# Takatsuka-Mark/Photogrammetry

Hardware: AMD Instinct MI355X
Metric: descriptor pairs matched/sec (higher is better)
Workload: dtype u8 / bits (descriptor bits expanded to fp4 +-1 for the MFMA distance: exact integers in f32 accumulators; integer keys); f32 grey; 1 GPU; BASELINE configs[2] (SURVEY 8d config 3) x 1: 64-frame 1920x1080 RGBA64 sequence(s), dewarp(shipped coeffs)+gray+FAST(T=0.1)+NMS(r=16; SURVEY 8d writes r = 20 for this config: both leave more than 4096 survivors per frame, the lists are cut to the same length either way)+BRIEF-256 per frame, all 2016 ordered image pairs per sequence through the greedy Hamming match, <=4096 keypoints per frame (fir; frames=64, image_pairs=2016, frames_per_gpu=64, image_pairs_per_gpu=2016, parallelism=frames f mod 1, image pairs p mod 1; 2 all-gathers per step (elided at N = 1), jobs_in_flight=2, rehearsal_on_one_gpu_with_gloo=False

## Files before the change

### photogrammetry_amd/csrc/k_brief.hip

```cpp
#include "pgx_internal.h"

namespace {

constexpr int MAX_WORDS = 128;

__device__ __forceinline__ void brief_256(const float *__restrict__ g, int W, int H, int x, int y,
                                          const int4 *__restrict__ pairs, uint32_t *__restrict__ out)
{
    const int lane = threadIdx.x & 63;
    int4 pr[4];
#pragma unroll
    for (int c = 0; c < 4; c++) pr[c] = pairs[c * 64 + lane];
    float v1[4], v2[4];
    bool ok[4];
#pragma unroll
    for (int c = 0; c < 4; c++) {
        const int x1 = x + pr[c].x, y1 = y + pr[c].y, x2 = x + pr[c].z, y2 = y + pr[c].w;
        ok[c] = x1 >= 0 && x1 < W && y1 >= 0 && y1 < H && x2 >= 0 && x2 < W && y2 >= 0 && y2 < H;
        v1[c] = ok[c] ? g[(size_t)y1 * W + x1] : 0.f;
        v2[c] = ok[c] ? g[(size_t)y2 * W + x2] : 0.f;
    }
    unsigned long long rev[4];
#pragma unroll
    for (int c = 0; c < 4; c++) rev[c] = __brevll(__ballot(ok[c] && v1[c] < v2[c]));
    if (lane < 8) {
        const int q = lane >> 1;
        const unsigned long long r = q == 0 ? rev[3] : (q == 1 ? rev[2] : (q == 2 ? rev[1] : rev[0]));
        out[lane] = (lane & 1) ? (uint32_t)(r >> 32) : (uint32_t)r;
    }
}

__device__ __forceinline__ void brief_one(const float *__restrict__ g, int W, int H, int x, int y,
                                          const int4 *__restrict__ pairs, int P, int words, uint32_t *wbuf ,
                                          uint32_t *__restrict__ out)
{
    const int lane = threadIdx.x & 63;
    for (int w = lane; w < words + 2; w += 64) wbuf[w] = 0;
    __builtin_amdgcn_wave_barrier();
    const int nchunk = (P + 63) / 64;
    for (int c = 0; c < nchunk; c++) {
        const int p = c * 64 + lane;
        bool bit = false;
        if (p < P) {
            const int4 pr = pairs[p];
            const int x1 = x + pr.x, y1 = y + pr.y;
            if (x1 >= 0 && x1 < W && y1 >= 0 && y1 < H) {
                const int x2 = x + pr.z, y2 = y + pr.w;
                if (x2 >= 0 && x2 < W && y2 >= 0 && y2 < H)
                    bit = g[(size_t)y1 * W + x1] < g[(size_t)y2 * W + x2];
            }
        }
        const unsigned long long rev = __brevll(__ballot(bit));
        if (lane == 0) {
            const int off = P - 64 * (c + 1);
            unsigned long long v = rev;
            int o = off;
            if (o < 0) { v >>= -o; o = 0; }
            const int wi = o >> 5, sh = o & 31;
            wbuf[wi] |= (uint32_t)(v << sh);
            wbuf[wi + 1] |= (uint32_t)(sh ? (v >> (32 - sh)) : (v >> 32));
            if (sh) wbuf[wi + 2] |= (uint32_t)(v >> (64 - sh));
        }
    }
    __builtin_amdgcn_wave_barrier();
    for (int w = lane; w < words; w += 64) out[w] = wbuf[w];
}

__global__ __launch_bounds__(256) void k_brief_kept(const float *__restrict__ gray, int W, int H,
                                                    const uint32_t *__restrict__ raw_xy,
                                                    const int32_t *__restrict__ raw_score, int raw_cap,
                                                    const uint32_t *__restrict__ order,
                                                    const int32_t *__restrict__ n_kept, int kp_cap,
                                                    const int4 *__restrict__ pairs, int P, int words,
                                                    pgx_keypoint *__restrict__ kp_out, uint32_t *__restrict__ desc_out,
                                                    int32_t *__restrict__ counts_out, int nframes, int out_stride)
{
    __shared__ uint32_t wbuf[4][MAX_WORDS + 2];
    const int nblk = (kp_cap + 3) / 4;
    const int F8 = (nframes / 8) * 8;
    int f, kb;
    {
        const int Lid = blockIdx.x;
        if (Lid < nblk * F8) {
            const int j = Lid >> 3;
            f = (j / nblk) * 8 + (Lid & 7);
            kb = j % nblk;
        } else {
            const int r = Lid - nblk * F8;
            f = F8 + r / nblk;
            kb = r % nblk;
        }
    }
    const int wv = threadIdx.x >> 6, lane = threadIdx.x & 63;
    const int k = kb * 4 + wv;
    const int nk = n_kept[f];
    if (kb == 0 && threadIdx.x == 0) counts_out[f] = nk;
    if (k >= nk) return;
    const uint32_t ri = order[(size_t)f * kp_cap + k];
    const uint32_t xy = raw_xy[(size_t)f * raw_cap + ri];
    const int x = (int)(xy & 0xFFFFu), y = (int)(xy >> 16);
    const float *g = gray + (size_t)f * W * H;
    if (lane == 0) {
        pgx_keypoint kp;
        kp.x = x; kp.y = y; kp.fast_score = raw_score[(size_t)f * raw_cap + ri];
        kp.value = g[(size_t)y * W + x];
        kp_out[(size_t)f * out_stride + k] = kp;
    }
    if (P == 256) brief_256(g, W, H, x, y, pairs, desc_out + ((size_t)f * out_stride + k) * 8);
    else brief_one(g, W, H, x, y, pairs, P, words, wbuf[wv], desc_out + ((size_t)f * out_stride + k) * words);
}

__global__ __launch_bounds__(256) void k_brief_list(const float *__restrict__ gray, int W, int H,
                                                    const pgx_keypoint *__restrict__ kps, int n,
                                                    const int4 *__restrict__ pairs, int P, int words,
                                                    uint32_t *__restrict__ desc_out)
{
    __shared__ uint32_t wbuf[4][MAX_WORDS + 2];
    const int wv = threadIdx.x >> 6;
    const int k = blockIdx.x * 4 + wv;
    if (k >= n) return;
    if (P == 256) brief_256(gray, W, H, kps[k].x, kps[k].y, pairs, desc_out + (size_t)k * 8);
    else brief_one(gray, W, H, kps[k].x, kps[k].y, pairs, P, words, wbuf[wv], desc_out + (size_t)k * words);
}

}

void pgx_launch_brief(hipStream_t s, const float *gray, int F, int W, int H, const uint32_t *raw_xy,
                      const int32_t *raw_score, int raw_cap, const uint32_t *order, const int32_t *n_kept,
                      int kp_cap, const int32_t *pairs, int P, pgx_keypoint *kp_out, uint32_t *desc_out,
                      int32_t *counts_out, int out_stride)
{
    if (F <= 0 || kp_cap <= 0) return;
    const int words = (P + 31) / 32;
    hipLaunchKernelGGL(k_brief_kept, dim3(((kp_cap + 3) / 4) * F), dim3(256), 0, s, gray, W, H, raw_xy, raw_score,
                       raw_cap, order, n_kept, kp_cap, reinterpret_cast<const int4 *>(pairs), P, words, kp_out,
                       desc_out, counts_out, F, out_stride);
}

void pgx_launch_brief_list(hipStream_t s, const float *gray, int W, int H, const pgx_keypoint *kps, int n,
                           const int32_t *pairs, int P, uint32_t *desc_out)
{
    if (n <= 0) return;
    const int words = (P + 31) / 32;
    hipLaunchKernelGGL(k_brief_list, dim3((n + 3) / 4), dim3(256), 0, s, gray, W, H, kps, n,
                       reinterpret_cast<const int4 *>(pairs), P, words, desc_out);
}
```

### photogrammetry_amd/csrc/pgx_api.hip

```cpp
#include "pgx_trackgraph.h"

#include <atomic>
#include <cmath>
#include <cstdarg>
#include <cstdio>
#include <new>
#include <cstring>
#include <cstdlib>

#define PGX_VERSION_STR "pgx 0.1 (gfx950)"

static thread_local std::string tl_err;
static thread_local const pgx_ctx *tl_err_ctx = nullptr;
static thread_local unsigned long long tl_err_id = 0;
static std::atomic<unsigned long long> g_ctx_ids{0};

void pgx_note_error(pgx_ctx *c, const std::string &msg)
{
    tl_err = msg;
    tl_err_ctx = c;
    tl_err_id = c ? c->id : 0;
    if (c) {
        std::lock_guard<std::mutex> g(c->err_mu);
        c->err = msg;
    }
}

namespace {

int fail(pgx_ctx *c, int code, const char *fmt, ...)
{
    char buf[512];
    va_list ap;
    va_start(ap, fmt);
    vsnprintf(buf, sizeof buf, fmt, ap);
    va_end(ap);
    pgx_note_error(c, buf);
    return code;
}

#define HIPCHK(c, expr)                                                                           \
    do {                                                                                          \
        hipError_t e_ = (expr);                                                                   \
        if (e_ != hipSuccess) return fail((c), PGX_E_HIP, "%s: %s", #expr, hipGetErrorString(e_)); \
    } while (0)

struct Lock {
    std::lock_guard<std::mutex> g;
    explicit Lock(pgx_ctx *c) : g(c->mu) { (void)hipSetDevice(c->device); }
};

int decode_status(pgx_ctx *c, int bits)
{
// ... 61 lines not shown
    if (dims_ok(c, W, H) != PGX_OK) return PGX_E_BADARG;
    if (c->map_set && (c->mapW != W || c->mapH != H))
        return fail(c, PGX_E_DIM_MISMATCH, "image %dx%d vs dewarp map %dx%d (ArgumentException)", W, H, c->mapW, c->mapH);
    if (F <= 0) return PGX_OK;
    const size_t npix = (size_t)W * H;
    const size_t nseg = pgx_fast_seg_count(W, H);
    const int raw_cap = c->raw_cap;
    HIPCHK(c, c->ws_gray.ensure((size_t)F * npix * 4));
    HIPCHK(c, c->ws_seg.ensure((size_t)F * nseg * 32));
    HIPCHK(c, c->ws_segoff.ensure((size_t)F * nseg * 4));
    HIPCHK(c, c->ws_rawxy.ensure((size_t)F * raw_cap * 4));
    HIPCHK(c, c->ws_rawscore.ensure((size_t)F * raw_cap * 4));
    const size_t nms_stride = pgx_nms_ws_bytes(W, H, c->radius, raw_cap, true);
    HIPCHK(c, c->ws_nms.ensure((size_t)F * nms_stride));
    const int kp_eff = c->kp_cap <= cap ? c->kp_cap : cap;
    HIPCHK(c, c->ws_order.ensure((size_t)F * kp_eff * 4));
    HIPCHK(c, c->ws_nkept.ensure((size_t)F * 4));
    return PGX_OK;
}

int pgx_enqueue_detect(pgx_ctx *c, const uint16_t *d_rgba, int F, int W, int H, pgx_keypoint *d_kp, uint32_t *d_desc,
                       int32_t *d_counts, int32_t *d_nraw, int cap)
{
    const int rcp = pgx_prepare_detect(c, F, W, H, cap);
    if (rcp != PGX_OK) return rcp;
    if (F <= 0) return PGX_OK;
    const int raw_cap = c->raw_cap;
    const size_t nms_stride = pgx_nms_ws_bytes(W, H, c->radius, raw_cap, true);
    const bool kp_soft = c->kp_cap <= cap;
    const int kp_eff = kp_soft ? c->kp_cap : cap;

    float *gray = c->ws_gray.as<float>();
    {
        ProfScope ps(c, "dewarp_gray");
        pgx_launch_dewarp_gray(c->stream, d_rgba, c->src8, c->map_set ? c->d_map.as<int32_t>() : nullptr, F, W, H, gray,
                               nullptr, c->d_status);
    }
    {
        ProfScope ps(c, "fast");
        pgx_launch_fast(c->stream, gray, F, W, H, c->threshold, c->ws_seg.as<unsigned long long>(),
                        c->ws_segoff.as<uint32_t>(), d_nraw, c->ws_rawxy.as<uint32_t>(),
                        c->ws_rawscore.as<int32_t>(), raw_cap, c->d_status,
                        !pgx_nms_fills_raw_lists(W, H, c->radius, raw_cap));
    }
    {
        ProfScope ps(c, "nms");
        pgx_launch_nms(c->stream, c->ws_rawxy.as<uint32_t>(), c->ws_rawscore.as<int32_t>(), d_nraw, F, raw_cap, W, H,
                       c->radius, c->ws_nms.p, nms_stride, c->ws_order.as<uint32_t>(), c->ws_nkept.as<int32_t>(),
                       kp_eff, c->d_status, c->ws_seg.as<unsigned long long>(), c->ws_segoff.as<uint32_t>(), kp_soft);
    }
    {
        ProfScope ps(c, "brief");
        pgx_launch_brief(c->stream, gray, F, W, H, c->ws_rawxy.as<uint32_t>(), c->ws_rawscore.as<int32_t>(), raw_cap,
                         c->ws_order.as<uint32_t>(), c->ws_nkept.as<int32_t>(), kp_eff, c->d_pairs.as<int32_t>(), c->P,
                         d_kp, d_desc, d_counts, cap);
    }
    HIPCHK(c, hipEventRecord(c->ev_stage[PGX_STAGE_DETECT], c->stream));
    HIPCHK(c, hipGetLastError());
    return PGX_OK;
}

int pgx_prepare_match(pgx_ctx *c, int stride, int words, int M)
{
    if (M <= 0) return PGX_OK;
    if (stride <= 0 || stride > (1 << PGX_IDX_BITS)) return fail(c, PGX_E_BADARG, "stride must be in [1, 2^20]");
    if (words <= 0 || words > 127) return fail(c, PGX_E_BADARG, "words must be in [1, 127] (P <= 4064)");
    const int CHUNK = c->match_chunk;
    const int mc = M < CHUNK ? M : CHUNK;
    const int nws = (M <= CHUNK || c->prof_serial || CHUNK >= PGX_PIPELINE_BELOW) ? 1 : 3;
    for (int k = 0; k < nws; k++) HIPCHK(c, c->ws_matchn[k].ensure(pgx_match_ws_bytes(mc, stride)));
    return PGX_OK;
}

int pgx_enqueue_match(pgx_ctx *c, const uint32_t *d_desc, const int32_t *d_counts, int stride, int words,
                      const int32_t *d_pairlist, int M, int max_n, pgx_pair *d_out)
{
    hipEvent_t gate = c->match_gate;
    c->match_gate = nullptr;
    if (M <= 0) return PGX_OK;
    const int rcp = pgx_prepare_match(c, stride, words, M);
    if (rcp != PGX_OK) return rcp;
    const int CHUNK = c->match_chunk;
    MatchPlan plan;
    plan.stride = stride; plan.words = words;
    plan.max_n = max_n > stride ? stride : (max_n < 1 ? 1 : max_n);
    plan.rounds_mfma = 0;
    plan.skip_below = words == 8 ? PGX_TAIL_MAX : PGX_TAIL_FILL_MAX;
    if (words == 8 && M <= 2) plan.skip_below = PGX_TAIL_MAX / 2;
    for (int n = plan.max_n; n > plan.skip_below && plan.rounds_mfma < PGX_MAX_WIDE_ROUNDS; n = (n + 1) / 2) plan.rounds_mfma++;
    if (plan.rounds_mfma > 0 && plan.rounds_mfma < PGX_MAX_WIDE_ROUNDS) plan.rounds_mfma++;
    HIPCHK(c, hipMemsetAsync(c->d_status + 4, 0, PGX_MAX_WIDE_ROUNDS * 8, c->stream));
    if (M <= CHUNK || c->prof_serial || CHUNK >= PGX_PIPELINE_BELOW) {
        for (int m0 = 0; m0 < M; m0 += CHUNK) {
            plan.M = (M - m0 < CHUNK) ? M - m0 : CHUNK;
            const int32_t *pl = d_pairlist + 2 * (size_t)m0;
            pgx_launch_match_wide(c, c->stream, d_desc, d_counts, pl, plan, c->ws_matchn[0].p, c->d_status, m0 == 0 ? gate : nullptr);
            const bool last = m0 + CHUNK >= M;
            if (last) HIPCHK(c, hipEventRecord(c->ev_stage[PGX_STAGE_MATCH_WIDE], c->stream));
            pgx_launch_match_rows(c, c->stream, d_desc, pl, plan, c->ws_matchn[0].p, c->d_status);
            if (last) HIPCHK(c, hipEventRecord(c->ev_stage[PGX_STAGE_MATCH_ROWS], c->stream));
            pgx_launch_match_finish(c, c->stream, d_desc, pl, plan, c->ws_matchn[0].p, d_out + (size_t)m0 * stride, c->d_status);
        }
    } else {
        const int NS = 3;
        int lo = 0, hi = 0;
        HIPCHK(c, hipDeviceGetStreamPriorityRange(&lo, &hi));
        for (int k = 0; k < NS; k++) {
// ... 37 lines not shown
    }
    c->last_rounds_mfma = plan.rounds_mfma;
    HIPCHK(c, hipEventRecord(c->ev_stage[PGX_STAGE_MATCH_DONE], c->stream));
    HIPCHK(c, hipGetLastError());
    return PGX_OK;
}

extern "C" {

const char *pgx_version(void) { return PGX_VERSION_STR; }

int pgx_ctx_create(int device, pgx_ctx **out)
{
    if (!out) return PGX_E_BADARG;
    *out = nullptr;
    int ndev = 0;
    if (hipGetDeviceCount(&ndev) != hipSuccess || ndev <= 0 || device < 0 || device >= ndev) return PGX_E_HIP;
    if (hipSetDevice(device) != hipSuccess) return PGX_E_HIP;
    hipDeviceProp_t prop;
    if (hipGetDeviceProperties(&prop, device) != hipSuccess) return PGX_E_HIP;
    if (strncmp(prop.gcnArchName, "gfx950", 6) != 0) {
        fprintf(stderr, "pgx: device %d is %s; this library is built for gfx950 only\n", device, prop.gcnArchName);
        return PGX_E_HIP;
    }
    pgx_ctx *c = new (std::nothrow) pgx_ctx();
    if (!c) return PGX_E_HIP;
    c->device = device;
    c->id = ++g_ctx_ids;
    if (hipStreamCreateWithFlags(&c->own_stream, hipStreamNonBlocking) != hipSuccess ||
        hipEventCreateWithFlags(&c->ev_stage[0], hipEventDisableTiming) != hipSuccess ||
        hipEventCreateWithFlags(&c->ev_stage[1], hipEventDisableTiming) != hipSuccess ||
        hipEventCreateWithFlags(&c->ev_stage[2], hipEventDisableTiming) != hipSuccess ||
        hipEventCreateWithFlags(&c->ev_stage[3], hipEventDisableTiming) != hipSuccess ||
        hipMalloc(reinterpret_cast<void **>(&c->d_status), 256) != hipSuccess ||
        hipHostMalloc(reinterpret_cast<void **>(&c->h_status), 64, hipHostMallocDefault) != hipSuccess ||
        hipMemset(c->d_status, 0, 256) != hipSuccess) {
        pgx_ctx_destroy(c);
        return PGX_E_HIP;
    }
    c->stream = c->own_stream;
    *out = c;
    return PGX_OK;
}

void pgx_ctx_destroy(pgx_ctx *c)
{
    if (!c) return;
    (void)hipSetDevice(c->device);
    if (c->stream) (void)hipStreamSynchronize(c->stream);
    if (c->comm) (void)pgx_comm_destroy(c);
    for (auto &kv : c->prof)
        for (auto &ev : kv.second.pending) { (void)hipEventDestroy(ev.first); (void)hipEventDestroy(ev.second); }
    for (hipEvent_t ev : c->ev_pool) (void)hipEventDestroy(ev);
    DevBuf *bufs[] = {&c->d_pairs, &c->d_map, &c->ws_gray, &c->ws_seg, &c->ws_segoff, &c->ws_nraw, &c->ws_rawxy,
                      &c->ws_rawscore, &c->ws_nms, &c->ws_order, &c->ws_nkept, &c->st_a, &c->st_b, &c->st_c,
                      &c->st_d, &c->st_e, &c->st_f, &c->ws_pose, &c->ws_tracks, &c->ws_tracks_split, &c->ws_agree, &c->ws_matchn[0], &c->ws_matchn[1], &c->ws_matchn[2], &c->ws_knn, &c->ws_guided, &c->ws_tri, &c->ws_ba, &c->ws_reg};
    for (DevBuf *b : bufs) b->release();
    c->pin_in.release();
    c->pin_out.release();
    if (c->d_status) (void)hipFree(c->d_status);
    if (c->h_status) (void)hipHostFree(c->h_status);
    for (int k = 0; k < 3; k++) {
        if (c->mstream[k]) (void)hipStreamDestroy(c->mstream[k]);
        if (c->ev_wide[k]) (void)hipEventDestroy(c->ev_wide[k]);
        if (c->ev_rows[k]) (void)hipEventDestroy(c->ev_rows[k]);
        if (c->ev_fin[k]) (void)hipEventDestroy(c->ev_fin[k]);
        if (c->ev_join[k]) (void)hipEventDestroy(c->ev_join[k]);
    }
    if (c->ev_in) (void)hipEventDestroy(c->ev_in);
    for (int k = 0; k < 4; k++) if (c->ev_stage[k]) (void)hipEventDestroy(c->ev_stage[k]);
    if (c->own_stream) (void)hipStreamDestroy(c->own_stream);
    delete c;
}

const char *pgx_last_error(pgx_ctx *c)
{
    if (!c) return "null context";
    if (tl_err_ctx == c && tl_err_id == c->id) return tl_err.c_str();
    static thread_local std::string copy;
    {
        std::lock_guard<std::mutex> g(c->err_mu);
        copy = c->err;
    }
    return copy.c_str();
}

int pgx_set_stream(pgx_ctx *c, void *hip_stream)
{
    if (!c) return PGX_E_BADARG;
    Lock l(c);
    c->cfg_epoch++;
    HIPCHK(c, hipStreamSynchronize(c->stream));
    c->stream = hip_stream ? reinterpret_cast<hipStream_t>(hip_stream) : c->own_stream;
    return PGX_OK;
}

int pgx_check_status(pgx_ctx *c)
{
    if (!c) return PGX_E_BADARG;
    Lock l(c);
    return sync_status(c);
}

int pgx_set_dewarp_map(pgx_ctx *c, const int32_t *uv, int W, int H)
{
    if (!c) return PGX_E_BADARG;
    Lock l(c);
    c->cfg_epoch++;
    if (!uv) { c->map_set = false; c->mapW = c->mapH = 0; return PGX_OK; }
    if (dims_ok(c, W, H, "map dimensions must fit ushort") != PGX_OK) return PGX_E_BADARG;
    const size_t bytes = (size_t)W * H * 8;
    HIPCHK(c, hipStreamSynchronize(c->stream));
    HIPCHK(c, c->d_map.ensure(bytes + 32));
    HIPCHK(c, hipMemcpy(c->d_map.p, uv, bytes, hipMemcpyHostToDevice));
    c->mapW = W; c->mapH = H; c->map_set = true;
    return PGX_OK;
}

int pgx_set_dewarp_coeffs(pgx_ctx *c, int W, int H, const double *coeffs, int ncoeffs)
{
    if (!c || !coeffs) return c ? fail(c, PGX_E_BADARG, "null pointer") : PGX_E_BADARG;
    Lock l(c);
    c->cfg_epoch++;
    if (ncoeffs != 5) return fail(c, PGX_E_BADARG, "You must pass exactly 5 distortion coefficients (ArgumentException)");
    if (dims_ok(c, W, H, "map dimensions must fit ushort") != PGX_OK) return PGX_E_BADARG;
    const size_t bytes = (size_t)W * H * 8;
    HIPCHK(c, hipStreamSynchronize(c->stream));
    HIPCHK(c, c->d_map.ensure(bytes + 32));
    pgx_launch_dewarp_map(c->stream, W, H, coeffs, c->d_map.as<int32_t>(), c->d_status);
    HIPCHK(c, hipGetLastError());
    c->mapW = W; c->mapH = H; c->map_set = true;
    return sync_status(c);
}

int pgx_get_dewarp_map(pgx_ctx *c, int32_t *uv_out, int W, int H)
{
    if (!c || !uv_out) return c ? fail(c, PGX_E_BADARG, "null pointer") : PGX_E_BADARG;
    Lock l(c);
    if (!c->map_set) return fail(c, PGX_E_NOT_CONFIGURED, "no dewarp map is set");
    if (W != c->mapW || H != c->mapH) return fail(c, PGX_E_DIM_MISMATCH, "map is %dx%d, asked for %dx%d", c->mapW, c->mapH, W, H);
    HIPCHK(c, hipStreamSynchronize(c->stream));
    HIPCHK(c, hipMemcpy(uv_out, c->d_map.p, (size_t)W * H * 8, hipMemcpyDeviceToHost));
    return PGX_OK;
}

int pgx_set_brief_pairs(pgx_ctx *c, const int32_t *pairs, int P)
{
    if (!c) return PGX_E_BADARG;
    Lock l(c);
    c->cfg_epoch++;
    if (!pairs || P <= 0 || P > 4064) return fail(c, PGX_E_BADARG, "P must be in [1, 4064]");
    HIPCHK(c, hipStreamSynchronize(c->stream));
    HIPCHK(c, c->d_pairs.ensure((size_t)P * 16));
    HIPCHK(c, hipMemcpy(c->d_pairs.p, pairs, (size_t)P * 16, hipMemcpyHostToDevice));
    c->P = P; c->words = (P + 31) / 32; c->pairs_set = true;
    return PGX_OK;
}

int pgx_set_detect_params(pgx_ctx *c, float threshold, int suppression_radius)
{
    if (!c) return PGX_E_BADARG;
    Lock l(c);
    c->cfg_epoch++;
    c->threshold = threshold; c->radius = suppression_radius; c->params_set = true;
    return PGX_OK;
}

int pgx_set_match_chunk(pgx_ctx *c, int pairs)
{
    if (!c) return PGX_E_BADARG;
    Lock l(c);
    c->cfg_epoch++;
    if (pairs < 16 || pairs > 4096) return fail(c, PGX_E_BADARG, "image pairs per chunk must be in [16, 4096]");
    c->match_chunk = pairs;
    return PGX_OK;
}

int pgx_wait_stage(pgx_ctx *c, pgx_ctx *other, int stage)
{
    if (!c || !other) return c ? fail(c, PGX_E_BADARG, "null context") : PGX_E_BADARG;
    Lock l(c);
    if (stage < 0 || stage > PGX_STAGE_MATCH_DONE) return fail(c, PGX_E_BADARG, "unknown stage %d", stage);
    if (c == other) return PGX_OK;
    if (c->device != other->device) return fail(c, PGX_E_BADARG, "contexts on different devices (%d, %d)", c->device, other->device);
    HIPCHK(c, hipStreamWaitEvent(c->stream, other->ev_stage[stage], 0));
    return PGX_OK;
}

int pgx_gate_match(pgx_ctx *c, pgx_ctx *other, int stage)
{
    if (!c || !other) return c ? fail(c, PGX_E_BADARG, "null context") : PGX_E_BADARG;
    Lock l(c);
    if (stage < 0 || stage > PGX_STAGE_MATCH_DONE) return fail(c, PGX_E_BADARG, "unknown stage %d", stage);
    if (c->device != other->device) return fail(c, PGX_E_BADARG, "contexts on different devices (%d, %d)", c->device, other->device);
    c->match_gate = c == other ? nullptr : other->ev_stage[stage];
    return PGX_OK;
}

int pgx_set_source_format(pgx_ctx *c, int format)
{
    if (!c) return PGX_E_BADARG;
    Lock l(c);
    c->cfg_epoch++;
    if (format != PGX_SRC_RGBA64 && format != PGX_SRC_RGBA8) return fail(c, PGX_E_BADARG, "unknown source format %d", format);
    c->src8 = format == PGX_SRC_RGBA8;
    return PGX_OK;
}
// ... 46 lines not shown
    if (!c || !gray || !n_out || (capacity > 0 && !out) || capacity < 0)
        return c ? fail(c, PGX_E_BADARG, "null pointer") : PGX_E_BADARG;
    Lock l(c);
    if (!c->params_set) return fail(c, PGX_E_NOT_CONFIGURED, "pgx_set_detect_params not called");
    if (dims_ok(c, W, H) != PGX_OK) return PGX_E_BADARG;
    const size_t npix = (size_t)W * H, nseg = pgx_fast_seg_count(W, H);
    const int cap = capacity > 0 ? capacity : 1;
    HIPCHK(c, c->st_a.ensure(npix * 4 + 32));
    HIPCHK(c, c->ws_seg.ensure(nseg * 32));
    HIPCHK(c, c->ws_segoff.ensure(nseg * 4));
    HIPCHK(c, c->ws_nraw.ensure(64));
    HIPCHK(c, c->st_b.ensure((size_t)cap * 4));
    HIPCHK(c, c->st_c.ensure((size_t)cap * 4));
    HIPCHK(c, hipMemcpyAsync(c->st_a.p, gray, npix * 4, hipMemcpyHostToDevice, c->stream));
    pgx_launch_fast(c->stream, c->st_a.as<float>(), 1, W, H, c->threshold, c->ws_seg.as<unsigned long long>(),
                    c->ws_segoff.as<uint32_t>(), c->ws_nraw.as<int32_t>(), c->st_b.as<uint32_t>(),
                    c->st_c.as<int32_t>(), cap, c->d_status);
    int n = 0;
    HIPCHK(c, hipMemcpyAsync(&n, c->ws_nraw.p, 4, hipMemcpyDeviceToHost, c->stream));
    int rc = sync_status(c);
    *n_out = n;
    const int nw = n < capacity ? n : capacity;
    if (nw > 0) {
        std::vector<uint32_t> xy(nw);
        std::vector<int32_t> sc(nw);
        HIPCHK(c, hipMemcpy(xy.data(), c->st_b.p, (size_t)nw * 4, hipMemcpyDeviceToHost));
        HIPCHK(c, hipMemcpy(sc.data(), c->st_c.p, (size_t)nw * 4, hipMemcpyDeviceToHost));
        for (int i = 0; i < nw; i++) {
            out[i].x = (int32_t)(xy[i] & 0xFFFFu);
            out[i].y = (int32_t)(xy[i] >> 16);
            out[i].fast_score = sc[i];
            out[i].value = gray[(size_t)out[i].y * W + out[i].x];
        }
    }
    if (rc == PGX_OK && n > capacity) return fail(c, PGX_E_CAPACITY, "%d hits, capacity %d", n, capacity);
    return rc;
}

int pgx_brief(pgx_ctx *c, const float *gray, int W, int H, const pgx_keypoint *kps, int n, uint32_t *desc_out)
{
    if (!c || !gray || n < 0 || (n > 0 && (!kps || !desc_out)))
        return c ? fail(c, PGX_E_BADARG, "null pointer") : PGX_E_BADARG;
    Lock l(c);
    if (!c->pairs_set) return fail(c, PGX_E_NOT_CONFIGURED, "pgx_set_brief_pairs not called");
    if (dims_ok(c, W, H) != PGX_OK) return PGX_E_BADARG;
    if (n == 0) return PGX_OK;
    const size_t npix = (size_t)W * H;
    HIPCHK(c, c->st_a.ensure(npix * 4 + 32));
    HIPCHK(c, c->st_b.ensure((size_t)n * sizeof(pgx_keypoint)));
    HIPCHK(c, c->st_c.ensure((size_t)n * c->words * 4));
    HIPCHK(c, hipMemcpyAsync(c->st_a.p, gray, npix * 4, hipMemcpyHostToDevice, c->stream));
    HIPCHK(c, hipMemcpyAsync(c->st_b.p, kps, (size_t)n * sizeof(pgx_keypoint), hipMemcpyHostToDevice, c->stream));
    pgx_launch_brief_list(c->stream, c->st_a.as<float>(), W, H, c->st_b.as<pgx_keypoint>(), n,
                          c->d_pairs.as<int32_t>(), c->P, c->st_c.as<uint32_t>());
    HIPCHK(c, hipMemcpyAsync(desc_out, c->st_c.p, (size_t)n * c->words * 4, hipMemcpyDeviceToHost, c->stream));
    return sync_status(c);
}

int pgx_nms(pgx_ctx *c, const pgx_keypoint *kps, int n, int W, int H, int32_t *order_out, int *n_out)
{
    if (!c || !n_out || n < 0 || (n > 0 && (!kps || !order_out)))
        return c ? fail(c, PGX_E_BADARG, "null pointer") : PGX_E_BADARG;
    Lock l(c);
    if (!c->params_set) return fail(c, PGX_E_NOT_CONFIGURED, "pgx_set_detect_params not called");
    if (dims_ok(c, W, H) != PGX_OK) return PGX_E_BADARG;
    *n_out = 0;
    if (n == 0) return PGX_OK;
    std::vector<uint32_t> xy(n);
    std::vector<int32_t> sc(n);
    for (int i = 0; i < n; i++) {
        if (kps[i].x < 0 || kps[i].x >= W || kps[i].y < 0 || kps[i].y >= H)
            return fail(c, PGX_E_BADARG, "keypoint %d (%d,%d) outside %dx%d", i, kps[i].x, kps[i].y, W, H);
        xy[i] = ((uint32_t)kps[i].y << 16) | (uint32_t)kps[i].x;
        sc[i] = kps[i].fast_score;
    }
    const size_t wsb = pgx_nms_ws_bytes(W, H, c->radius, n, false);
    HIPCHK(c, c->st_a.ensure((size_t)n * 4));
    HIPCHK(c, c->st_b.ensure((size_t)n * 4));
    HIPCHK(c, c->st_c.ensure((size_t)n * 4));
    HIPCHK(c, c->st_d.ensure(64));
    HIPCHK(c, c->ws_nms.ensure(wsb));
    HIPCHK(c, hipMemcpyAsync(c->st_a.p, xy.data(), (size_t)n * 4, hipMemcpyHostToDevice, c->stream));
    HIPCHK(c, hipMemcpyAsync(c->st_b.p, sc.data(), (size_t)n * 4, hipMemcpyHostToDevice, c->stream));
    HIPCHK(c, hipMemcpyAsync(c->st_d.p, &n, 4, hipMemcpyHostToDevice, c->stream));
    HIPCHK(c, pgx_launch_nms_sync(c->stream, c->st_a.as<uint32_t>(), c->st_b.as<int32_t>(), c->st_d.as<int32_t>(), n, W, H,
                                  c->radius, c->ws_nms.p, wsb, c->st_c.as<uint32_t>(), c->st_d.as<int32_t>() + 1, n,
                                  c->d_status));
    int nk = 0;
    HIPCHK(c, hipMemcpyAsync(&nk, c->st_d.as<int32_t>() + 1, 4, hipMemcpyDeviceToHost, c->stream));
    int rc = sync_status(c);
    if (rc != PGX_OK) return rc;
    *n_out = nk;
    if (nk > 0) HIPCHK(c, hipMemcpy(order_out, c->st_c.p, (size_t)nk * 4, hipMemcpyDeviceToHost));
    return PGX_OK;
}

namespace {

struct TwoSets {
    int32_t meta[13];
    const uint32_t *desc;
    const pgx_keypoint *kp;
    const int32_t *counts, *pairlist;
    const float *F;
};
int stage_two_sets(pgx_ctx *c, const uint32_t *desc1, const pgx_keypoint *kp1, int n1, const uint32_t *desc2, const pgx_keypoint *kp2,
                   int n2, int S, int words, const float *F, TwoSets &d)
// ... 824 lines not shown
```

### photogrammetry_amd/csrc/pgx_internal.h

```cpp
#pragma once

#include <hip/hip_runtime.h>
#include <stdint.h>

#include <map>
#include <mutex>
#include <string>
#include <type_traits>
#include <utility>
#include <vector>

#include "../../include/pgx.h"

#define PGX_ST_OOB_SOURCE 1u
#define PGX_ST_RAW_CAP    2u
#define PGX_ST_KP_CAP     4u
#define PGX_ST_EMPTY_SET  8u
#define PGX_ST_INTERNAL   16u
#define PGX_ST_BADARG     32u
#define PGX_ST_DUP_FRAME  64u
#define PGX_ST_TRI_CAP    128u
#define PGX_ST_TRI_NODE   256u
#define PGX_ST_TRI_DUP    512u
#define PGX_ST_BA_CAP     1024u
// ... 18 lines not shown

struct DevBuf {
    void *p = nullptr;
    size_t cap = 0;
    hipError_t ensure(size_t bytes)
    {
        if (bytes <= cap) return hipSuccess;
        if (p) { hipError_t e = hipFree(p); p = nullptr; cap = 0; if (e != hipSuccess) return e; }
        size_t want = bytes + bytes / 4 + 256;
        hipError_t e = hipMalloc(&p, want);
        if (e == hipSuccess) cap = want;
        return e;
    }
    void release() { if (p) (void)hipFree(p); p = nullptr; cap = 0; }
    template <class T> T *as() const { return reinterpret_cast<T *>(p); }
};

struct PinBuf {
    void *p = nullptr;
    size_t cap = 0;
    hipError_t ensure(size_t bytes)
    {
        if (bytes <= cap) return hipSuccess;
        if (p) { (void)hipHostFree(p); p = nullptr; cap = 0; }
        const size_t want = bytes + bytes / 4 + 4096;
        hipError_t e = hipHostMalloc(&p, want, hipHostMallocDefault);
        if (e == hipSuccess) cap = want;
        return e;
    }
    void release() { if (p) (void)hipHostFree(p); p = nullptr; cap = 0; }
    template <class T> T *as() const { return reinterpret_cast<T *>(p); }
};

struct ProfEntry {
    std::vector<std::pair<hipEvent_t, hipEvent_t>> pending;
    int launches = 0;
    double total_ms = 0.0;
};

struct pgx_ctx {
    int device = 0;
    hipStream_t own_stream = nullptr;
    hipStream_t stream = nullptr;
    std::mutex mu;
    std::string err;
    std::mutex err_mu;

    float threshold = 0.f;
    int radius = 0;
    bool params_set = false;
    int P = 0, words = 0;
    bool pairs_set = false;
    DevBuf d_pairs;
    int mapW = 0, mapH = 0;
    bool map_set = false;
    DevBuf d_map;
    int raw_cap = 1 << 17;
    int kp_cap = 1 << PGX_IDX_BITS;
    int match_chunk = 2048;
    int src8 = 0;

    int *d_status = nullptr;
    int *h_status = nullptr;

    DevBuf ws_gray, ws_seg, ws_segoff, ws_nraw, ws_rawxy, ws_rawscore, ws_nms, ws_order, ws_nkept;
    DevBuf st_a, st_b, st_c, st_d, st_e, st_f;
    PinBuf pin_in, pin_out;
    DevBuf ws_matchn[3];
    DevBuf ws_pose, ws_tracks;
    DevBuf ws_tracks_split;
    DevBuf ws_knn;
    DevBuf ws_guided;
    DevBuf ws_tri;
    DevBuf ws_ba;
    DevBuf ws_reg;
    hipStream_t mstream[3] = {nullptr, nullptr, nullptr};
    hipEvent_t ev_in = nullptr, ev_wide[3] = {nullptr, nullptr, nullptr}, ev_rows[3] = {nullptr, nullptr, nullptr},
               ev_fin[3] = {nullptr, nullptr, nullptr}, ev_join[3] = {nullptr, nullptr, nullptr};
    hipEvent_t ev_stage[4] = {nullptr, nullptr, nullptr, nullptr};
    hipEvent_t match_gate = nullptr;

    void *comm = nullptr;
    int comm_rank = 0, comm_world = 1;
    std::string comm_agreed;
    unsigned cfg_epoch = 0;
    unsigned long long id = 0;
    DevBuf ws_agree;

    bool prof_on = false;
    std::string prof_only;
    bool prof_serial = false;
    std::map<std::string, ProfEntry> prof;
    std::vector<hipEvent_t> ev_pool;

    int last_rounds_mfma = 0;
    long long last_evals = 0;
};

#ifdef __HIPCC__
__host__ __device__ __forceinline__ unsigned long long *pgx_dbg(int *status) { return reinterpret_cast<unsigned long long *>(status + PGX_DBG_OFF); }
__device__ __forceinline__ void pgx_xcd_map(int lin, int nblk, int F, int &f, int &b)
{
    const int F8 = (F >> 3) << 3;
    if (lin < nblk * F8) {
        const int j = lin >> 3;
        f = (j / nblk) * 8 + (lin & 7);
// ... 11 lines not shown
struct ProfScope {
    pgx_ctx *c;
    ProfEntry *e = nullptr;
    hipEvent_t a = nullptr, b = nullptr;
    hipStream_t st;
    bool attach;
    ProfScope(pgx_ctx *ctx, const char *name, hipStream_t s = nullptr, bool attach_to_kernel = false)
        : c(ctx), st(s ? s : ctx->stream), attach(attach_to_kernel)
    {
        if (!name || !c->prof_on || (!c->prof_only.empty() && c->prof_only != name)) return;
        e = &c->prof[name];
        auto take = [&](hipEvent_t &ev) {
            if (!c->ev_pool.empty()) { ev = c->ev_pool.back(); c->ev_pool.pop_back(); return true; }
            return hipEventCreate(&ev) == hipSuccess;
        };
        if (!take(a) || !take(b)) { e = nullptr; a = b = nullptr; return; }
        if (!attach) (void)hipEventRecord(a, st);
    }
    ~ProfScope()
    {
        if (!e) return;
        if (!attach) (void)hipEventRecord(b, st);
        e->pending.emplace_back(a, b);
    }
};


void pgx_launch_dewarp_gray(hipStream_t s, const void *rgba, int src8, const int32_t *map_uv, int F, int W, int H,
                            float *gray, uint16_t *dewarped, int *status);
void pgx_launch_dewarp_map(hipStream_t s, int W, int H, const double *k , int32_t *map_uv, int *status);

size_t pgx_fast_seg_count(int W, int H);
void pgx_launch_fast(hipStream_t s, const float *gray, int F, int W, int H, float T,
                     unsigned long long *seg , uint32_t *segoff ,
                     int32_t *n_raw , uint32_t *raw_xy ,
                     int32_t *raw_score , int raw_cap, int *status,
                     bool compact = true );

size_t pgx_nms_ws_bytes(int W, int H, int radius, int n_cap, bool planes);
bool pgx_nms_fills_raw_lists(int W, int H, int radius, int n_cap);
void pgx_launch_nms(hipStream_t s, uint32_t *raw_xy, int32_t *raw_score, const int32_t *n_raw,
                    int F, int n_cap, int W, int H, int radius, void *ws, size_t ws_stride,
                    uint32_t *order , int32_t *n_kept , int kp_cap, int *status,
                    const unsigned long long *seg = nullptr ,
                    const uint32_t *segoff = nullptr,
                    bool kp_soft = false );
hipError_t pgx_launch_nms_sync(hipStream_t s, const uint32_t *raw_xy, const int32_t *raw_score, const int32_t *n_raw,
                               int n_cap, int W, int H, int radius, void *ws, size_t ws_stride, uint32_t *order,
                               int32_t *n_kept, int kp_cap, int *status);

void pgx_launch_brief(hipStream_t s, const float *gray, int F, int W, int H,
                      const uint32_t *raw_xy, const int32_t *raw_score, int raw_cap,
                      const uint32_t *order, const int32_t *n_kept, int kp_cap ,
                      const int32_t *pairs, int P,
                      pgx_keypoint *kp_out, uint32_t *desc_out, int32_t *counts_out, int out_stride );
void pgx_launch_brief_list(hipStream_t s, const float *gray, int W, int H, const pgx_keypoint *kps, int n,
                           const int32_t *pairs, int P, uint32_t *desc_out);

size_t pgx_pose_ws_bytes(int M, int n_samples);
void pgx_launch_fundamental(hipStream_t s, const pgx_keypoint *kp, const pgx_pair *matches, const int32_t *counts,
                            const int32_t *pairlist, int M, int stride, int n_samples, int P, float threshold, int rank_check,
                            uint64_t seed, void *ws, float *F_out, int32_t *inliers, int32_t *best_sample);
void pgx_launch_pose(hipStream_t s, const pgx_keypoint *kp, const pgx_pair *matches, const int32_t *counts,
                     const int32_t *pairlist, int M, int stride, const float *F_in, float *Rt_out, int32_t *votes,
                     int32_t *best, float *points);

size_t pgx_tracks_ws_bytes(int n_frames, int stride);
void pgx_launch_tracks(hipStream_t s, const pgx_pair *d_matches, const int32_t *d_counts, const int32_t *d_pairlist, int M, int F,
                       int stride, const int32_t *d_frame_ids, int n_frames, int max_dist, int min_len, void *ws,
                       int32_t *d_track_of, int32_t *d_offsets, int32_t *d_nodes, int32_t *d_summary);
size_t pgx_tracks_split_ws_bytes(int n_frames, int stride);
void pgx_launch_tracks_split(hipStream_t s, const pgx_pair *d_matches, const int32_t *d_counts, const int32_t *d_pairlist, int M,
                             int F, int stride, const int32_t *d_frame_ids, int n_frames, int max_dist, const int *gates,
                             int n_gates, int min_len, void *ws, int32_t *d_track_of, int32_t *d_offsets, int32_t *d_nodes,
                             int32_t *d_summary, int *status);

struct MatchPlan {
    int M;
    int stride;
    int words;
    int max_n;
    int rounds_mfma;
    int skip_below = PGX_TAIL_FILL_MAX;
};
size_t pgx_match_ws_bytes(int M, int stride);
void pgx_launch_match_wide(pgx_ctx *ctx, hipStream_t s, const uint32_t *d_desc, const int32_t *d_counts,
                           const int32_t *d_pairlist, const MatchPlan &plan, void *ws, int *status, hipEvent_t gate = nullptr);
void pgx_launch_match_rows(pgx_ctx *ctx, hipStream_t s, const uint32_t *d_desc, const int32_t *d_pairlist,
                           const MatchPlan &plan, void *ws, int *status);
void pgx_launch_match_finish(pgx_ctx *ctx, hipStream_t s, const uint32_t *d_desc, const int32_t *d_pairlist,
                             const MatchPlan &plan, void *ws, pgx_pair *d_out, int *status);

void pgx_launch_knn(pgx_ctx *ctx, hipStream_t s, const uint32_t *d_desc, const int32_t *d_counts, const int32_t *d_pairlist, int M,
                    int S, int words, int max_n, int k, int32_t *d_idx, int32_t *d_dist, int32_t *d_col);
void pgx_launch_colkeys(pgx_ctx *ctx, hipStream_t s, const char *scope, bool finish, const int32_t *d_counts,
                        const int32_t *d_pairlist, int M, int S, int max_n, int32_t *d_col);
void pgx_launch_knn_select(pgx_ctx *ctx, hipStream_t s, const int32_t *d_counts, const int32_t *d_pairlist, int M, int S, int max_n,
                           const int32_t *d_idx, const int32_t *d_dist, const int32_t *d_col, int max_dist, float ratio,
                           int cross_check, pgx_pair *d_out);

size_t pgx_guided_ws_bytes(int M, int max_n);
void pgx_launch_guided(pgx_ctx *ctx, hipStream_t s, const uint32_t *d_desc, const pgx_keypoint *d_kp, const int32_t *d_counts,
                       const int32_t *d_pairlist, int M, int S, int words, int max_n, const float *d_F, float band, int k,
                       int32_t *d_idx, int32_t *d_dist, int32_t *d_col, void *ws, int *status);

size_t pgx_triangulate_ws_bytes(int n_frames);
void pgx_launch_triangulate(hipStream_t s, const pgx_keypoint *d_kp, int F, int stride, const int32_t *d_frame_ids, int n_frames,
                            const double *d_P, const int32_t *d_offsets, const int32_t *d_nodes, long long node_cap,
                            const int32_t *d_track_summary, int max_tracks, double min_parallax_deg, double max_reproj_px,
                            int refine_iters, double *d_xyz, double *d_quality, int32_t *d_flags, double *d_node_err,
// ... 17 lines not shown
```

Measured before the change: 4837 billion descriptor pairs/s.

## Gather BRIEF samples in row-sorted order through an LDS strip

For 256-pair BRIEF, a host-built plan sorts the 512 sample offsets by row and column. Each wave gathers pixels in that sorted order, so neighbouring lanes touch nearby addresses, and stores values plus in-bounds masks in an LDS strip. The pair comparisons then read those values back via per-pair index words. This targets scattered global gathers in the descriptor stage, at the cost of more LDS per block and a wave barrier. The metric is matching throughput, so the BRIEF stage may carry little weight in it.

Result: faster. 5092 billion descriptor pairs/s, median of 6 (+5.3%).

```diff
diff --git a/photogrammetry_amd/csrc/k_brief.hip b/photogrammetry_amd/csrc/k_brief.hip
--- a/photogrammetry_amd/csrc/k_brief.hip
+++ b/photogrammetry_amd/csrc/k_brief.hip
@@ -1,28 +1,54 @@
 #include "pgx_internal.h"
+#include "pgx_brief_plan.h"
 
 namespace {
 
 constexpr int MAX_WORDS = 128;
 
-__device__ __forceinline__ void brief_256(const float *__restrict__ g, int W, int H, int x, int y,
-                                          const int4 *__restrict__ pairs, uint32_t *__restrict__ out)
+constexpr int STRIP_WORDS = PGX_PLAN_SAMPLES + 16;
+static_assert(MAX_WORDS + 2 <= STRIP_WORDS && PGX_PLAN_PAIRS == 256, "the LDS strip also serves brief_one");
+
+__device__ __forceinline__ void brief_256(const float *__restrict__ img, int W, int H, int x, int y,
+                                          const int32_t *__restrict__ plan, uint32_t *strip ,
+                                          uint32_t *__restrict__ out)
 {
     const int lane = threadIdx.x & 63;
-    int4 pr[4];
+    const int2 *smp = reinterpret_cast<const int2 *>(plan);
+    const uint32_t *pos = reinterpret_cast<const uint32_t *>(plan) + 2 * PGX_PLAN_SAMPLES;
+    float *val = reinterpret_cast<float *>(strip);
+    uint32_t *mask = strip + PGX_PLAN_SAMPLES;
+    int2 sm[8];
 #pragma unroll
-    for (int c = 0; c < 4; c++) pr[c] = pairs[c * 64 + lane];
-    float v1[4], v2[4];
-    bool ok[4];
+    for (int g = 0; g < 8; g++) sm[g] = smp[g * 64 + lane];
+    uint32_t off[8];
+    bool in[8];
+#pragma unroll
+    for (int g = 0; g < 8; g++) {
+        const int xs = x + sm[g].x, ys = y + sm[g].y;
+        in[g] = xs >= 0 && xs < W && ys >= 0 && ys < H;
+        off[g] = (uint32_t)ys * (uint32_t)W + (uint32_t)xs;
+        const unsigned long long m = __ballot(in[g]);
+        if (lane == 0) { mask[2 * g] = (uint32_t)m; mask[2 * g + 1] = (uint32_t)(m >> 32); }
+    }
+    float v[8];
+#pragma unroll
+    for (int g = 0; g < 8; g++) v[g] = in[g] ? img[off[g]] : 0.f;
+    uint32_t pp[4];
+#pragma unroll
+    for (int c = 0; c < 4; c++) pp[c] = pos[c * 64 + lane];
+#pragma unroll
+    for (int g = 0; g < 8; g++) val[g * 64 + lane] = v[g];
+    __builtin_amdgcn_fence(__ATOMIC_RELEASE, "wavefront");
+    __builtin_amdgcn_wave_barrier();
+    __builtin_amdgcn_fence(__ATOMIC_ACQUIRE, "wavefront");
+    unsigned long long rev[4];
 #pragma unroll
     for (int c = 0; c < 4; c++) {
-        const int x1 = x + pr[c].x, y1 = y + pr[c].y, x2 = x + pr[c].z, y2 = y + pr[c].w;
-        ok[c] = x1 >= 0 && x1 < W && y1 >= 0 && y1 < H && x2 >= 0 && x2 < W && y2 >= 0 && y2 < H;
-        v1[c] = ok[c] ? g[(size_t)y1 * W + x1] : 0.f;
-        v2[c] = ok[c] ? g[(size_t)y2 * W + x2] : 0.f;
+        const uint32_t p1 = pp[c] & 511u, p2 = (pp[c] >> 16) & 511u;
+        const bool ok = ((mask[p1 >> 5] >> (p1 & 31)) & (mask[p2 >> 5] >> (p2 & 31)) & 1u) != 0;
+        const float v1 = val[p1], v2 = val[p2];
+        rev[c] = __brevll(__ballot(ok && v1 < v2));
     }
-    unsigned long long rev[4];
-#pragma unroll
-    for (int c = 0; c < 4; c++) rev[c] = __brevll(__ballot(ok[c] && v1[c] < v2[c]));
     if (lane < 8) {
         const int q = lane >> 1;
         const unsigned long long r = q == 0 ? rev[3] : (q == 1 ? rev[2] : (q == 2 ? rev[1] : rev[0]));
@@ -66,16 +92,17 @@
     for (int w = lane; w < words; w += 64) out[w] = wbuf[w];
 }
 
+template <bool P256>
 __global__ __launch_bounds__(256) void k_brief_kept(const float *__restrict__ gray, int W, int H,
                                                     const uint32_t *__restrict__ raw_xy,
                                                     const int32_t *__restrict__ raw_score, int raw_cap,
                                                     const uint32_t *__restrict__ order,
                                                     const int32_t *__restrict__ n_kept, int kp_cap,
-                                                    const int4 *__restrict__ pairs, int P, int words,
-                                                    pgx_keypoint *__restrict__ kp_out, uint32_t *__restrict__ desc_out,
+                                                    const int4 *__restrict__ pairs, const int32_t *__restrict__ plan, int P,
+                                                    int words, pgx_keypoint *__restrict__ kp_out, uint32_t *__restrict__ desc_out,
                                                     int32_t *__restrict__ counts_out, int nframes, int out_stride)
 {
-    __shared__ uint32_t wbuf[4][MAX_WORDS + 2];
+    __shared__ uint32_t wbuf[4][STRIP_WORDS];
     const int nblk = (kp_cap + 3) / 4;
     const int F8 = (nframes / 8) * 8;
     int f, kb;
@@ -106,20 +133,21 @@
         kp.value = g[(size_t)y * W + x];
         kp_out[(size_t)f * out_stride + k] = kp;
     }
-    if (P == 256) brief_256(g, W, H, x, y, pairs, desc_out + ((size_t)f * out_stride + k) * 8);
+    if (P256) brief_256(g, W, H, x, y, plan, wbuf[wv], desc_out + ((size_t)f * out_stride + k) * 8);
     else brief_one(g, W, H, x, y, pairs, P, words, wbuf[wv], desc_out + ((size_t)f * out_stride + k) * words);
 }
 
+template <bool P256>
 __global__ __launch_bounds__(256) void k_brief_list(const float *__restrict__ gray, int W, int H,
                                                     const pgx_keypoint *__restrict__ kps, int n,
-                                                    const int4 *__restrict__ pairs, int P, int words,
-                                                    uint32_t *__restrict__ desc_out)
+                                                    const int4 *__restrict__ pairs, const int32_t *__restrict__ plan, int P,
+                                                    int words, uint32_t *__restrict__ desc_out)
 {
-    __shared__ uint32_t wbuf[4][MAX_WORDS + 2];
+    __shared__ uint32_t wbuf[4][STRIP_WORDS];
     const int wv = threadIdx.x >> 6;
     const int k = blockIdx.x * 4 + wv;
     if (k >= n) return;
-    if (P == 256) brief_256(gray, W, H, kps[k].x, kps[k].y, pairs, desc_out + (size_t)k * 8);
+    if (P256) brief_256(gray, W, H, kps[k].x, kps[k].y, plan, wbuf[wv], desc_out + (size_t)k * 8);
     else brief_one(gray, W, H, kps[k].x, kps[k].y, pairs, P, words, wbuf[wv], desc_out + (size_t)k * words);
 }
 
@@ -127,21 +155,21 @@
 
 void pgx_launch_brief(hipStream_t s, const float *gray, int F, int W, int H, const uint32_t *raw_xy,
                       const int32_t *raw_score, int raw_cap, const uint32_t *order, const int32_t *n_kept,
-                      int kp_cap, const int32_t *pairs, int P, pgx_keypoint *kp_out, uint32_t *desc_out,
+                      int kp_cap, const int32_t *pairs, const int32_t *plan, int P, pgx_keypoint *kp_out, uint32_t *desc_out,
                       int32_t *counts_out, int out_stride)
 {
     if (F <= 0 || kp_cap <= 0) return;
     const int words = (P + 31) / 32;
-    hipLaunchKernelGGL(k_brief_kept, dim3(((kp_cap + 3) / 4) * F), dim3(256), 0, s, gray, W, H, raw_xy, raw_score,
-                       raw_cap, order, n_kept, kp_cap, reinterpret_cast<const int4 *>(pairs), P, words, kp_out,
+    hipLaunchKernelGGL(P == PGX_PLAN_PAIRS ? k_brief_kept<true> : k_brief_kept<false>, dim3(((kp_cap + 3) / 4) * F), dim3(256), 0, s, gray, W, H, raw_xy, raw_score,
+                       raw_cap, order, n_kept, kp_cap, reinterpret_cast<const int4 *>(pairs), plan, P, words, kp_out,
                        desc_out, counts_out, F, out_stride);
 }
 
 void pgx_launch_brief_list(hipStream_t s, const float *gray, int W, int H, const pgx_keypoint *kps, int n,
-                           const int32_t *pairs, int P, uint32_t *desc_out)
+                           const int32_t *pairs, const int32_t *plan, int P, uint32_t *desc_out)
 {
     if (n <= 0) return;
     const int words = (P + 31) / 32;
-    hipLaunchKernelGGL(k_brief_list, dim3((n + 3) / 4), dim3(256), 0, s, gray, W, H, kps, n,
-                       reinterpret_cast<const int4 *>(pairs), P, words, desc_out);
+    hipLaunchKernelGGL(P == PGX_PLAN_PAIRS ? k_brief_list<true> : k_brief_list<false>, dim3((n + 3) / 4), dim3(256), 0, s, gray, W, H, kps, n,
+                       reinterpret_cast<const int4 *>(pairs), plan, P, words, desc_out);
 }
diff --git a/photogrammetry_amd/csrc/pgx_api.hip b/photogrammetry_amd/csrc/pgx_api.hip
--- a/photogrammetry_amd/csrc/pgx_api.hip
+++ b/photogrammetry_amd/csrc/pgx_api.hip
@@ -1,4 +1,5 @@
 #include "pgx_trackgraph.h"
+#include "pgx_brief_plan.h"
 
 #include <atomic>
 #include <cmath>
@@ -166,7 +167,7 @@
     {
         ProfScope ps(c, "brief");
         pgx_launch_brief(c->stream, gray, F, W, H, c->ws_rawxy.as<uint32_t>(), c->ws_rawscore.as<int32_t>(), raw_cap,
-                         c->ws_order.as<uint32_t>(), c->ws_nkept.as<int32_t>(), kp_eff, c->d_pairs.as<int32_t>(), c->P,
+                         c->ws_order.as<uint32_t>(), c->ws_nkept.as<int32_t>(), kp_eff, c->d_pairs.as<int32_t>(), c->d_plan.as<int32_t>(), c->P,
                          d_kp, d_desc, d_counts, cap);
     }
     HIPCHK(c, hipEventRecord(c->ev_stage[PGX_STAGE_DETECT], c->stream));
@@ -310,7 +311,7 @@
     for (auto &kv : c->prof)
         for (auto &ev : kv.second.pending) { (void)hipEventDestroy(ev.first); (void)hipEventDestroy(ev.second); }
     for (hipEvent_t ev : c->ev_pool) (void)hipEventDestroy(ev);
-    DevBuf *bufs[] = {&c->d_pairs, &c->d_map, &c->ws_gray, &c->ws_seg, &c->ws_segoff, &c->ws_nraw, &c->ws_rawxy,
+    DevBuf *bufs[] = {&c->d_pairs, &c->d_plan, &c->d_map, &c->ws_gray, &c->ws_seg, &c->ws_segoff, &c->ws_nraw, &c->ws_rawxy,
                       &c->ws_rawscore, &c->ws_nms, &c->ws_order, &c->ws_nkept, &c->st_a, &c->st_b, &c->st_c,
                       &c->st_d, &c->st_e, &c->st_f, &c->ws_pose, &c->ws_tracks, &c->ws_tracks_split, &c->ws_agree, &c->ws_matchn[0], &c->ws_matchn[1], &c->ws_matchn[2], &c->ws_knn, &c->ws_guided, &c->ws_tri, &c->ws_ba, &c->ws_reg};
     for (DevBuf *b : bufs) b->release();
@@ -411,6 +412,12 @@
     HIPCHK(c, hipStreamSynchronize(c->stream));
     HIPCHK(c, c->d_pairs.ensure((size_t)P * 16));
     HIPCHK(c, hipMemcpy(c->d_pairs.p, pairs, (size_t)P * 16, hipMemcpyHostToDevice));
+    if (P == PGX_PLAN_PAIRS) {
+        int32_t plan[PGX_PLAN_WORDS];
+        pgx_build_brief_plan(pairs, plan);
+        HIPCHK(c, c->d_plan.ensure(sizeof plan));
+        HIPCHK(c, hipMemcpy(c->d_plan.p, plan, sizeof plan, hipMemcpyHostToDevice));
+    }
     c->P = P; c->words = (P + 31) / 32; c->pairs_set = true;
     return PGX_OK;
 }
@@ -563,7 +570,7 @@
     HIPCHK(c, hipMemcpyAsync(c->st_a.p, gray, npix * 4, hipMemcpyHostToDevice, c->stream));
     HIPCHK(c, hipMemcpyAsync(c->st_b.p, kps, (size_t)n * sizeof(pgx_keypoint), hipMemcpyHostToDevice, c->stream));
     pgx_launch_brief_list(c->stream, c->st_a.as<float>(), W, H, c->st_b.as<pgx_keypoint>(), n,
-                          c->d_pairs.as<int32_t>(), c->P, c->st_c.as<uint32_t>());
+                          c->d_pairs.as<int32_t>(), c->d_plan.as<int32_t>(), c->P, c->st_c.as<uint32_t>());
     HIPCHK(c, hipMemcpyAsync(desc_out, c->st_c.p, (size_t)n * c->words * 4, hipMemcpyDeviceToHost, c->stream));
     return sync_status(c);
 }
diff --git a/photogrammetry_amd/csrc/pgx_brief_plan.h b/photogrammetry_amd/csrc/pgx_brief_plan.h
--- /dev/null
+++ b/photogrammetry_amd/csrc/pgx_brief_plan.h
@@ -0,0 +1,25 @@
+#pragma once
+#include <algorithm>
+#include <cstdint>
+
+constexpr int PGX_PLAN_PAIRS = 256;
+constexpr int PGX_PLAN_SAMPLES = 2 * PGX_PLAN_PAIRS;
+constexpr int PGX_PLAN_WORDS = 2 * PGX_PLAN_SAMPLES + PGX_PLAN_PAIRS;
+
+inline void pgx_build_brief_plan(const int32_t *pairs , int32_t *plan )
+{
+    uint16_t idx[PGX_PLAN_SAMPLES];
+    for (int i = 0; i < PGX_PLAN_SAMPLES; i++) idx[i] = (uint16_t)i;
+    std::stable_sort(idx, idx + PGX_PLAN_SAMPLES, [pairs](uint16_t a, uint16_t b) {
+        const int32_t ax = pairs[2 * a], ay = pairs[2 * a + 1], bx = pairs[2 * b], by = pairs[2 * b + 1];
+        return ay != by ? ay < by : ax < bx;
+    });
+    uint32_t *pos = reinterpret_cast<uint32_t *>(plan + 2 * PGX_PLAN_SAMPLES);
+    for (int p = 0; p < PGX_PLAN_PAIRS; p++) pos[p] = 0;
+    for (int s = 0; s < PGX_PLAN_SAMPLES; s++) {
+        const int e = idx[s];
+        plan[2 * s] = pairs[2 * e];
+        plan[2 * s + 1] = pairs[2 * e + 1];
+        pos[e >> 1] |= (uint32_t)s << ((e & 1) * 16);
+    }
+}
diff --git a/photogrammetry_amd/csrc/pgx_internal.h b/photogrammetry_amd/csrc/pgx_internal.h
--- a/photogrammetry_amd/csrc/pgx_internal.h
+++ b/photogrammetry_amd/csrc/pgx_internal.h
@@ -94,6 +94,7 @@
     int P = 0, words = 0;
     bool pairs_set = false;
     DevBuf d_pairs;
+    DevBuf d_plan;
     int mapW = 0, mapH = 0;
     bool map_set = false;
     DevBuf d_map;
@@ -211,10 +212,10 @@
 void pgx_launch_brief(hipStream_t s, const float *gray, int F, int W, int H,
                       const uint32_t *raw_xy, const int32_t *raw_score, int raw_cap,
                       const uint32_t *order, const int32_t *n_kept, int kp_cap ,
-                      const int32_t *pairs, int P,
+                      const int32_t *pairs, const int32_t *plan , int P,
                       pgx_keypoint *kp_out, uint32_t *desc_out, int32_t *counts_out, int out_stride );
 void pgx_launch_brief_list(hipStream_t s, const float *gray, int W, int H, const pgx_keypoint *kps, int n,
-                           const int32_t *pairs, int P, uint32_t *desc_out);
+                           const int32_t *pairs, const int32_t *plan, int P, uint32_t *desc_out);
 
 size_t pgx_pose_ws_bytes(int M, int n_samples);
 void pgx_launch_fundamental(hipStream_t s, const pgx_keypoint *kp, const pgx_pair *matches, const int32_t *counts,
```
